# snowiow/SIFT

Measured on AMD Instinct MI355X. Metric: keypoints/sec, 1920x1080 4oct/3DoG, higher is better.
Workload: dtype f32

## Files before the change

### sift_amd/csrc/kernels_desc.hip

```cpp
#include <cstdio>

#include "common.h"
#include "hist_bins.h"

#pragma clang fp contract(off)

namespace sift_hip {

__device__ __forceinline__ int reflect_idx(int p, int n) {
    p = p < 0 ? -p : p;
    p = p >= n ? 2 * (n - 1) - p : p;
    return p < 0 ? 0 : (p >= n ? n - 1 : p);
}

__global__ __launch_bounds__(256) void w16_kernel(const float* __restrict__ level, float* __restrict__ w16,
                                                  int w, int h, const float* __restrict__ taps, int r) {
    const int img = blockIdx.x;
    const float* __restrict__ src = level + (size_t)img * (size_t)w * (size_t)h;
    const int lx = threadIdx.x & 15, ly = threadIdx.x >> 4;
    float out = 0.0f;
    if (lx < w && ly < h) {
        float sum = 0.0f;
        for (int t = 0; t <= 2 * r; ++t) {
            const int yy = reflect_idx(ly - r + t, h);
            float row = 0.0f;
            for (int s = 0; s <= 2 * r; ++s) {
                const int xx = reflect_idx(lx - r + s, w);
                row += taps[2 * r - s] * src[(size_t)yy * (size_t)w + (size_t)xx];
            }
            sum += taps[2 * r - t] * row;
        }
        out = sum;
    }
    w16[(size_t)img * 256 + (size_t)(lx + 16 * ly)] = out;
}

constexpr int kCellShift = 4;
constexpr int kW16Stride = 46;
constexpr int kW16Bias = 15 * kW16Stride + 15;
constexpr int kW16Size = 46 * kW16Stride;
struct W16Entry { float w; unsigned mask; };

typedef float f4u __attribute__((ext_vector_type(4), aligned(4)));

struct DescGridLevel {
    int w, h, dogs;
    int cw, ch, cell_base, cells_per_image;
    const float* mag;
    const float* ori;
    const float* gauss;
    const float* w16;
    int* wire_sums;
};

__device__ __forceinline__ int desc_cell_of(const DevPlan* __restrict__ plan, const FinalKp& f, int& level) {
    const int D = plan->dogs;
    level = plan->nearest_level[f.octave * D + f.index];
    const int o = level / (D + 1);
    const int w = plan->w[o], h = plan->h[o];
    const int kx = f.x, ky = f.y;
    if (kx < kRegion || kx > w - kRegion || ky < kRegion || ky > h - kRegion) return -1;
    return plan->desc_cell_base[level] + (ky >> kCellShift) * plan->desc_cw[level] + (kx >> kCellShift);
}

constexpr int kGridThreads = 1024;
constexpr int kGridLdsCells = 16384;

template <bool LDS_COUNTS>
__global__ __launch_bounds__(kGridThreads) void desc_grid_kernel(const DevPlan* __restrict__ plan, const FinalKp* __restrict__ finals,
                                                                 const int* __restrict__ final_cnt, int final_cap,
                                                                 int* __restrict__ cell_cnt, int* __restrict__ cell_off,
                                                                 FinalKp* __restrict__ pool, int pool_cap,
                                                                 long long* out_base, int compute_base,
                                                                 sift_hip_keypoint* __restrict__ kp_out, float* __restrict__ desc_out,
                                                                 long long out_cap) {
    __shared__ int s_cnt[LDS_COUNTS ? kGridLdsCells : 1];
    __shared__ int s_part[kGridThreads];
    __shared__ long long s_wsum[kGridThreads / 64];
    const int img = blockIdx.x, tid = threadIdx.x;
    const int K = final_cnt[img];
    long long my_base;
    if (compute_base) {
        long long sum = 0;
        for (int i = tid; i < img; i += kGridThreads) sum += final_cnt[i];
#pragma unroll
        for (int o = 32; o > 0; o >>= 1) sum += __shfl_down(sum, o);
        if ((tid & 63) == 0) s_wsum[tid >> 6] = sum;
        __syncthreads();
        long long t = 0;
#pragma unroll
        for (int wv = 0; wv < kGridThreads / 64; ++wv) t += s_wsum[wv];
        my_base = t;
        if (tid == 0) out_base[img] = t;
    } else {
        my_base = out_base[img];
    }
    const int cpi = plan->desc_cells_per_image;
    int* cnt = LDS_COUNTS ? s_cnt : cell_cnt + (size_t)img * (size_t)(cpi + 1);
    int* off = cell_off + (size_t)img * (size_t)(cpi + 1);
    const FinalKp* __restrict__ fin = finals + (size_t)img * (size_t)final_cap;
    for (int i = tid; i < cpi; i += kGridThreads) cnt[i] = 0;
    __syncthreads();
    for (int k = tid; k < K; k += kGridThreads) {
        const FinalKp f = fin[k];
        int level;
        const int cell = desc_cell_of(plan, f, level);
        if (cell >= 0) {
            atomicAdd(&cnt[cell], 1);
        } else {
            const long long ok = my_base + k;
            if (ok < out_cap) {
                sift_hip_keypoint r;
                r.scale = plan->dog_scale[f.octave * plan->dogs + f.index];
                r.orientation = f.orientation;
                r.x = f.x; r.y = f.y; r.octave = f.octave; r.index = f.index;
                r.filtered = 1; r.has_descriptor = 0; r.reserved = 0;
                kp_out[ok] = r;
                float4* d = reinterpret_cast<float4*>(desc_out + (size_t)ok * 128);
                for (int i = 0; i < 32; ++i) d[i] = make_float4(0.0f, 0.0f, 0.0f, 0.0f);
            }
        }
    }
    __syncthreads();
    const int chunk = (cpi + kGridThreads - 1) / kGridThreads;
    const int lo = tid * chunk, hi = min(lo + chunk, cpi);
    int sum = 0;
    for (int i = lo; i < hi; ++i) sum += cnt[i];
    s_part[tid] = sum;
    __syncthreads();
    for (int o = 1; o < kGridThreads; o <<= 1) {
        const int v = tid >= o ? s_part[tid - o] : 0;
        __syncthreads();
        s_part[tid] += v;
        __syncthreads();
    }
    int run = s_part[tid] - sum;
    for (int i = lo; i < hi; ++i) {
        const int v = cnt[i];
        off[i] = run;
        cnt[i] = run;
        run += v;
    }
    if (tid == kGridThreads - 1) off[cpi] = s_part[kGridThreads - 1];
    __syncthreads();
    FinalKp* pl = pool + (size_t)img * (size_t)pool_cap;
    for (int k = tid; k < K; k += kGridThreads) {
        FinalKp f = fin[k];
        int level;
        const int cell = desc_cell_of(plan, f, level);
        if (cell < 0) continue;
        f.cand = (uint32_t)k;
        pl[atomicAdd(&cnt[cell], 1)] = f;
    }
}

__device__ __forceinline__ int wave_min_nonneg(int v) {
    v = min(v, __builtin_amdgcn_update_dpp(0x7fffffff, v, 0xB1, 0xf, 0xf, false));
    v = min(v, __builtin_amdgcn_update_dpp(0x7fffffff, v, 0x4E, 0xf, 0xf, false));
    v = min(v, __builtin_amdgcn_update_dpp(0x7fffffff, v, 0x141, 0xf, 0xf, false));
    v = min(v, __builtin_amdgcn_update_dpp(0x7fffffff, v, 0x140, 0xf, 0xf, false));
    return min(min(__builtin_amdgcn_readlane(v, 0), __builtin_amdgcn_readlane(v, 16)),
               min(__builtin_amdgcn_readlane(v, 32), __builtin_amdgcn_readlane(v, 48)));
}

template <int Y>
__device__ __forceinline__ float quad_bcast_f(float v) {
    return __uint_as_float((unsigned)__builtin_amdgcn_mov_dpp((int)__float_as_uint(v), Y * 0x55, 0xF, 0xF, true));
}
template <int Y>
__device__ __forceinline__ unsigned quad_bcast_u(unsigned v) {
    return (unsigned)__builtin_amdgcn_mov_dpp((int)v, Y * 0x55, 0xF, 0xF, true);
}
__device__ __forceinline__ float quad_prev_f(float v) {
    return __uint_as_float((unsigned)__builtin_amdgcn_mov_dpp((int)__float_as_uint(v), 0x93 , 0xF, 0xF, true));
}

#define SIFT_HIST_SAMPLE(Y)                                                                                  \
    "v_cmp_eq_u32_sdwa vcc, %[p], %[b0] src0_sel:BYTE_" #Y " src1_sel:DWORD\n\t"                              \
    "v_add_f32_dpp %[t], %[v], %[h0] quad_perm:[" #Y "," #Y "," #Y "," #Y "] row_mask:0xf bank_mask:0xf\n\t"  \
    "v_cndmask_b32 %[h0], %[h0], %[t], vcc\n\t"                                                               \
    "v_cmp_eq_u32_sdwa vcc, %[p], %[b1] src0_sel:BYTE_" #Y " src1_sel:DWORD\n\t"                              \
    "v_add_f32_dpp %[t], %[v], %[h1] quad_perm:[" #Y "," #Y "," #Y "," #Y "] row_mask:0xf bank_mask:0xf\n\t"  \
    "v_cndmask_b32 %[h1], %[h1], %[t], vcc\n\t"
__device__ __forceinline__ void cell_histograms(const float (&val)[4], const unsigned (&bin)[4], int lane, unsigned b0, unsigned b1,
                                                float& h0, float& h1) {
    const unsigned sh = 8u * (unsigned)(lane & 3);
    unsigned pk[4];
#pragma unroll
    for (int i = 0; i < 4; ++i) pk[i] = bin[i] << sh;
    asm volatile(
        "s_nop 1\n\t"
        "v_or_b32_dpp %[p0], %[p0], %[p0] quad_perm:[1,0,3,2] row_mask:0xf bank_mask:0xf\n\t"
        "v_or_b32_dpp %[p1], %[p1], %[p1] quad_perm:[1,0,3,2] row_mask:0xf bank_mask:0xf\n\t"
        "v_or_b32_dpp %[p2], %[p2], %[p2] quad_perm:[1,0,3,2] row_mask:0xf bank_mask:0xf\n\t"
        "v_or_b32_dpp %[p3], %[p3], %[p3] quad_perm:[1,0,3,2] row_mask:0xf bank_mask:0xf\n\t"
        "v_or_b32_dpp %[p0], %[p0], %[p0] quad_perm:[2,3,0,1] row_mask:0xf bank_mask:0xf\n\t"
        "v_or_b32_dpp %[p1], %[p1], %[p1] quad_perm:[2,3,0,1] row_mask:0xf bank_mask:0xf\n\t"
        "v_or_b32_dpp %[p2], %[p2], %[p2] quad_perm:[2,3,0,1] row_mask:0xf bank_mask:0xf\n\t"
        "v_or_b32_dpp %[p3], %[p3], %[p3] quad_perm:[2,3,0,1] row_mask:0xf bank_mask:0xf\n\t"
        : [p0] "+v"(pk[0]), [p1] "+v"(pk[1]), [p2] "+v"(pk[2]), [p3] "+v"(pk[3]));
    float t;
#pragma unroll
    for (int i = 0; i < 4; ++i)
        asm volatile(
            "s_nop 1\n\t"
            SIFT_HIST_SAMPLE(0) SIFT_HIST_SAMPLE(1) SIFT_HIST_SAMPLE(2) SIFT_HIST_SAMPLE(3)
            : [h0] "+v"(h0), [h1] "+v"(h1), [t] "=&v"(t)
            : [p] "v"(pk[i]), [v] "v"(val[i]), [b0] "v"(b0), [b1] "v"(b1)
            : "vcc");
}
#undef SIFT_HIST_SAMPLE

__global__ __launch_bounds__(256, 8) void descriptor_wave_kernel(const DevPlan* __restrict__ plan, DescGridLevel lv,
                                                                 const int* __restrict__ cell_off,
                                                                 const FinalKp* __restrict__ pool, int pool_cap,
                                                                 const long long* __restrict__ out_base,
                                                                 sift_hip_keypoint* __restrict__ kp_out,
                                                                 float* __restrict__ desc_out, long long out_cap, int n_images,
                                                                 int chunks, int dbg_arg) {
    const int dbg = dbg_arg & kDiagMask;
    __shared__ __attribute__((aligned(8))) W16Entry s_w16t[kW16Size];
    __shared__ __attribute__((aligned(16))) uint2 s_list[4][64];
    __shared__ __attribute__((aligned(16))) unsigned s_keys[4][68];
    const int tid = threadIdx.x, lane = tid & 63;
    const int wave = __builtin_amdgcn_readfirstlane(tid >> 6);
    const int w = lv.w, h = lv.h, D = lv.dogs;
    const int ly = lane & 15, lx0 = (lane >> 4) * 4;
    const int tbase = kW16Bias + lx0 * kW16Stride + ly;
    const unsigned b0 = 2u * (unsigned)(lane & 3), b1 = b0 + 1u;
    for (int i = tid; i < kW16Size; i += 256) s_w16t[i] = W16Entry{0.0f, 0u};
    const int xcd = (int)blockIdx.x & 7, slot = (int)blockIdx.x >> 3, nslots = (int)gridDim.x >> 3;
    for (int unit = xcd; unit < n_images * chunks; unit += 8) {
    const int img = unit / chunks, chunk = unit - img * chunks;
    const int* __restrict__ coff = cell_off + (size_t)img * (size_t)(lv.cells_per_image + 1) + lv.cell_base;
    const int r_begin = coff[0], r_count = coff[lv.cw * lv.ch] - r_begin;
    const int e_begin = r_begin + (int)((long long)r_count * chunk / chunks), e_end = r_begin + (int)((long long)r_count * (chunk + 1) / chunks);
    if (e_begin + slot * 4 >= e_end) continue;
    __syncthreads();
    s_w16t[kW16Bias + (tid & 15) * kW16Stride + (tid >> 4)] = W16Entry{lv.w16[(size_t)img * 256 + tid], 0xffffffffu};
    __syncthreads();
    float wself[4];
#pragma unroll
    for (int i = 0; i < 4; ++i) wself[i] = s_w16t[tbase + i * kW16Stride].w;
    const size_t img_off = (size_t)img * (size_t)w * (size_t)h;
    const float* __restrict__ gm = lv.mag + img_off;
    const float* __restrict__ go = lv.ori + img_off;
    const float* __restrict__ gg = lv.gauss + img_off;
    const FinalKp* __restrict__ pl = pool + (size_t)img * (size_t)pool_cap;
    const long long obase = out_base[img];

    const int estride = nslots * 4;
    const int e0 = e_begin + slot * 4 + wave;
    struct Rec { int k; float theta; unsigned xy, oi; };
    struct Ranges { int s0, s1, s2, n0, n1, n2; };
    struct Window { f4u o, m, g; };
    auto load_rec = [&](int e) {
        const uint4 v = *reinterpret_cast<const uint4*>(&pl[min(e, e_end - 1)]);
        Rec r;
        r.k = (int)v.x; r.theta = __uint_as_float(v.y); r.xy = v.z; r.oi = v.w;
        return r;
    };
    auto load_ranges = [&](unsigned xy) {
        const int ccx = (int)(xy & 0xffffu) >> kCellShift, ccy = (int)(xy >> 16) >> kCellShift;
        const int c0 = max(ccx - 1, 0), c1 = min(ccx + 1, lv.cw - 1);
        const int y0 = max(ccy - 1, 0), y2 = min(ccy + 1, lv.ch - 1);
        const int a0 = coff[y0 * lv.cw + c0], b0_ = coff[y0 * lv.cw + c1 + 1];
        const int a1 = coff[ccy * lv.cw + c0], b1_ = coff[ccy * lv.cw + c1 + 1];
        const int a2 = coff[y2 * lv.cw + c0], b2_ = coff[y2 * lv.cw + c1 + 1];
        Ranges g;
        g.s0 = a0; g.n0 = ccy - 1 >= 0 ? b0_ - a0 : 0;
        g.s1 = a1; g.n1 = b1_ - a1;
        g.s2 = a2; g.n2 = ccy + 1 < lv.ch ? b2_ - a2 : 0;
        return g;
    };
    auto uniform_rec = [](const Rec& r) {
        Rec u;
        u.k = __builtin_amdgcn_readfirstlane(r.k);
        u.theta = __uint_as_float((unsigned)__builtin_amdgcn_readfirstlane((int)__float_as_uint(r.theta)));
        u.xy = (unsigned)__builtin_amdgcn_readfirstlane((int)r.xy);
        u.oi = (unsigned)__builtin_amdgcn_readfirstlane((int)r.oi);
        return u;
    };
    auto load_window = [&](unsigned xy) {
        size_t o = (size_t)((int)(xy >> 16) - kRegion + ly) * (size_t)w + (size_t)((int)(xy & 0xffffu) - kRegion + lx0);
        if (dbg & 8) o &= ~(size_t)3;
        if (dbg & 128) o = (size_t)ly * (size_t)w + (size_t)lx0 + (size_t)((xy >> 4) & 0xfffu) * 16u;
        Window wd;
        wd.o = (f4u)(1.0f); wd.m = (f4u)(2.0f); wd.g = (f4u)(3.0f);
        if (!(dbg & 4)) {
            wd.o = *reinterpret_cast<const f4u*>(go + o);
            wd.m = *reinterpret_cast<const f4u*>(gm + o);
            wd.g = *reinterpret_cast<const f4u*>(gg + o);
        }
        return wd;
    };
    auto entry_of = [](const Ranges& g, int i) {
        return i < g.n0 ? g.s0 + i : (i < g.n0 + g.n1 ? g.s1 + (i - g.n0) : g.s2 + (i - g.n0 - g.n1));
    };
    auto load_cand = [&](const Ranges& g) {
        const int T = g.n0 + g.n1 + g.n2;
        uint4 c = make_uint4(0u, 0u, 0u, 0u);
        if (lane < T && T <= 64) c = *reinterpret_cast<const uint4*>(&pl[entry_of(g, lane)]);
        return c;
    };
    Rec u0 = uniform_rec(load_rec(e0));
    Rec r1 = load_rec(e0 + estride);
    Ranges g0 = load_ranges(u0.xy);

    for (int e = e0; e < e_end; e += estride) {
        const uint4 c0v = load_cand(g0);
        const Window w0 = load_window(u0.xy);
        const Rec u1 = uniform_rec(r1);
        r1 = load_rec(e + 2 * estride);
        const Ranges g1 = load_ranges(u1.xy);
        const int myk = u0.k;
        const float mytheta = u0.theta;
        const unsigned myoi = u0.oi;
        const int px = (int)(u0.xy & 0xffffu), py = (int)(u0.xy >> 16);
        const int T = g0.n0 + g0.n1 + g0.n2;
        const uint4 c = c0v;
        float vo[4] = {w0.o.x, w0.o.y, w0.o.z, w0.o.w}, vm[4] = {w0.m.x, w0.m.y, w0.m.z, w0.m.w};
        const float vg[4] = {w0.g.x, w0.g.y, w0.g.z, w0.g.w};

        struct Wq { W16Entry v[4]; };
        auto weights_at = [&](int toff) {
            Wq r;
#pragma unroll
            for (int i = 0; i < 4; ++i) r.v[i] = s_w16t[tbase + toff + i * kW16Stride];
            return r;
        };
        auto apply_w = [&](unsigned qtheta_bits, const Wq& wq) {
#pragma unroll
            for (int i = 0; i < 4; ++i) {
                vo[i] = vo[i] + __uint_as_float(qtheta_bits & wq.v[i].mask);
                vm[i] = vm[i] + wq.v[i].w;
            }
        };
        auto apply = [&](unsigned qxy, float qtheta) {
            const int dx = px - (int)(qxy & 0xffffu), dy = py - (int)(qxy >> 16);
            apply_w(__float_as_uint(qtheta), weights_at(dx * kW16Stride + dy));
        };

        if (!(dbg & 1)) {
            auto precedes = [&](const uint4& c) {
                const int qx = (int)(c.z & 0xffffu), qy = (int)(c.z >> 16);
                return (int)c.x < myk && (unsigned)(qx - px + 15) < 31u && (unsigned)(qy - py + 15) < 31u;
            };
            if (T <= 64) {
                const bool pass = lane < T && precedes(c);
                const unsigned long long todo = __ballot(pass);
                const int n_prev = __popcll(todo);
                if (n_prev) {
                    unsigned* keys = s_keys[wave];
                    const int pos = (int)__builtin_amdgcn_mbcnt_hi((unsigned)(todo >> 32), __builtin_amdgcn_mbcnt_lo((unsigned)todo, 0u));
                    if (pass) keys[pos] = c.x;
                    if (lane < 4) keys[n_prev + lane] = 0xffffffffu;
                    __builtin_amdgcn_wave_barrier();
                    int rank = 0;
                    for (int ch = 0; ch < n_prev; ch += 4) {
                        const uint4 k4 = *reinterpret_cast<const uint4*>(keys + ch);
                        rank += (k4.x < c.x ? 1 : 0) + (k4.y < c.x ? 1 : 0) + (k4.z < c.x ? 1 : 0) + (k4.w < c.x ? 1 : 0);
                    }
                    uint2* list = s_list[wave];
                    if (pass) {
                        const int dx = px - (int)(c.z & 0xffffu), dy = py - (int)(c.z >> 16);
                        list[rank] = make_uint2(c.y, (unsigned)(dx * kW16Stride + dy));
                    }
                    __builtin_amdgcn_wave_barrier();
                    int r = 0;
                    for (; r + 1 < n_prev; r += 2) {
                        const uint4 q01 = *reinterpret_cast<const uint4*>(&list[r]);
                        const Wq wq0 = weights_at((int)q01.y), wq1 = weights_at((int)q01.w);
                        apply_w(q01.x, wq0);
                        apply_w(q01.z, wq1);
                    }
                    if (r < n_prev) {
                        const uint2 q0 = list[r];
                        apply_w(q0.x, weights_at((int)q0.y));
                    }
                    __builtin_amdgcn_wave_barrier();
                }
            } else {
                int last = -1;
                for (;;) {
                    int bk = 0x7fffffff;
                    unsigned bxy = 0u, bth = 0u;
                    for (int base = 0; base < T; base += 64) {
                        const int i = base + lane;
                        if (i < T) {
                            const uint4 c = *reinterpret_cast<const uint4*>(&pl[entry_of(g0, i)]);
                            if (precedes(c) && (int)c.x > last && (int)c.x < bk) { bk = (int)c.x; bxy = c.z; bth = c.y; }
                        }
                    }
                    const int m = wave_min_nonneg(bk);
                    if (m == 0x7fffffff) break;
                    const int src = (int)__builtin_ctzll(__ballot(bk == m));
                    apply((unsigned)__builtin_amdgcn_readlane((int)bxy, src), __uint_as_float((unsigned)__builtin_amdgcn_readlane((int)bth, src)));
                    last = m;
                }
            }
        }
        float val[4];
        unsigned bin[4];
#pragma unroll
        for (int i = 0; i < 4; ++i) {
            const float no = vo[i] + mytheta;
            const float nm = vm[i] + wself[i];
            val[i] = nm * vg[i];
            bin[i] = hist8_bin(no);
        }
        float h0 = 0.0f, h1 = 0.0f;
        if (!(dbg & 2)) {
            cell_histograms(val, bin, lane, b0, b1, h0, h1);
            float run = 0.0f;
            run += h0; run += h1;
            float acc = run;
#pragma unroll
            for (int step = 1; step < 4; ++step) {
                const float prev = quad_prev_f(acc);
                float t = prev;
                t += h0; t += h1;
                acc = ((lane & 3) == step) ? t : acc;
            }
            const float length = quad_bcast_f<3>(acc);
            if (!(length == 0.0f)) {
                h0 = h0 / length;
                h1 = h1 / length;
            }
        }
        const long long ok = obase + (long long)myk;
        if (ok < out_cap && !((dbg & 16) && h0 == 12345.0f)) {
            typedef float f2nt __attribute__((ext_vector_type(2)));
            __builtin_nontemporal_store((f2nt){h0, h1}, reinterpret_cast<f2nt*>(desc_out + (size_t)ok * 128 + (size_t)(2 * lane)));
            if (lv.wire_sums != nullptr) {
                const bool b0 = __float_as_uint(h0) != 0u, odd7 = (lane & 3) == 3;
                const bool b1 = !odd7 && __float_as_uint(h1) != 0u;
                const int nset = __popcll(__ballot(b0)) + __popcll(__ballot(b1));
                const unsigned long long bin7 = __ballot(odd7 && __float_as_uint(h1) != 0u);
                if (lane == 0) {
                    atomicAdd(&lv.wire_sums[1 + (ok >> 6)], nset);
                    if (bin7 != 0ull) atomicOr(&lv.wire_sums[0], 1);
                }
            }
            if (lane == 0) {
                sift_hip_keypoint r;
                r.scale = plan->dog_scale[(myoi & 0xffffu) * (unsigned)D + (myoi >> 16)];
                r.orientation = mytheta;
                r.x = (uint16_t)px; r.y = (uint16_t)py;
                r.octave = (uint16_t)(myoi & 0xffffu); r.index = (uint16_t)(myoi >> 16);
                r.filtered = 0; r.has_descriptor = 1; r.reserved = 0;
                kp_out[ok] = r;
            }
        }
        u0 = u1;
        g0 = g1;
    }
    }
}

void launch_w16(hipStream_t s, const DevPlan& plan, int level, const float* d_taps16, int radius16) {
    const int oct = level / (plan.dogs + 1);
    hipLaunchKernelGGL(w16_kernel, dim3((unsigned)plan.n_images), dim3(256), 0, s,
                       (const float*)plan.gauss[level], plan.w16[level], plan.w[oct], plan.h[oct], d_taps16,
                       radius16);
}

void launch_desc_grid(hipStream_t s, const DevPlan* d_plan, const DevPlan& plan, const FinalKp* d_final, const int* d_final_cnt,
                      int final_cap, int* d_cell_cnt, int* d_cell_off, FinalKp* d_pool, int pool_cap, long long* d_out_base,
                      bool compute_base, sift_hip_keypoint* d_kp_out, float* d_desc_out, long long out_cap) {
    if (plan.desc_cells_per_image <= kGridLdsCells)
        hipLaunchKernelGGL(desc_grid_kernel<true>, dim3((unsigned)plan.n_images), dim3(kGridThreads), 0, s, d_plan, d_final, d_final_cnt,
                           final_cap, d_cell_cnt, d_cell_off, d_pool, pool_cap, d_out_base, compute_base ? 1 : 0, d_kp_out, d_desc_out, out_cap);
    else
        hipLaunchKernelGGL(desc_grid_kernel<false>, dim3((unsigned)plan.n_images), dim3(kGridThreads), 0, s, d_plan, d_final, d_final_cnt,
                           final_cap, d_cell_cnt, d_cell_off, d_pool, pool_cap, d_out_base, compute_base ? 1 : 0, d_kp_out, d_desc_out, out_cap);
}

void launch_descriptors_wave(hipStream_t s, const DevPlan* d_plan, const DevPlan& plan, int level, const int* d_cell_off,
                             const FinalKp* d_pool, int pool_cap, const long long* d_out_base, sift_hip_keypoint* d_kp_out,
                             float* d_desc_out, long long out_cap, int dbg, int* d_wire_sums, hipEvent_t ev_start, hipEvent_t ev_stop) {
    DescGridLevel lv;
    const int oct = level / (plan.dogs + 1);
    lv.w = plan.w[oct]; lv.h = plan.h[oct]; lv.dogs = plan.dogs;
    lv.cw = plan.desc_cw[level]; lv.ch = plan.desc_ch[level]; lv.cell_base = plan.desc_cell_base[level];
    lv.cells_per_image = plan.desc_cells_per_image;
    lv.mag = plan.mag[level]; lv.ori = plan.ori[level]; lv.gauss = plan.gauss[level]; lv.w16 = plan.w16[level];
    lv.wire_sums = d_wire_sums;
    const int chunks = plan.n_images >= 8 ? 1 : 8;
    const unsigned nwg = (dbg & kDiagMask & 64) ? 512u : ((dbg & kDiagMask & 32) ? 1024u : 2048u);
    hipExtLaunchKernelGGL(descriptor_wave_kernel, dim3(nwg), dim3(256), 0, s, ev_start, ev_stop, 0, d_plan, lv, d_cell_off, d_pool, pool_cap, d_out_base,
                       d_kp_out, d_desc_out, out_cap, plan.n_images, chunks, dbg);
}

__global__ void tu_probe_desc_kernel() {}
void tu_touch_desc(hipStream_t s) { hipLaunchKernelGGL(tu_probe_desc_kernel, dim3(1), dim3(1), 0, s); }

}
```

Before: 230.4 million.

## Build per-cell orientation histograms in LDS instead of DPP compare-select chains

```diff
diff --git a/sift_amd/csrc/kernels_desc.hip b/sift_amd/csrc/kernels_desc.hip
--- a/sift_amd/csrc/kernels_desc.hip
+++ b/sift_amd/csrc/kernels_desc.hip
@@ -2,6 +2,7 @@
 
 #include "common.h"
 #include "hist_bins.h"
+#include "lds_tile.h"
 
 #pragma clang fp contract(off)
 
@@ -163,53 +164,42 @@
                min(__builtin_amdgcn_readlane(v, 32), __builtin_amdgcn_readlane(v, 48)));
 }
 
-template <int Y>
-__device__ __forceinline__ float quad_bcast_f(float v) {
-    return __uint_as_float((unsigned)__builtin_amdgcn_mov_dpp((int)__float_as_uint(v), Y * 0x55, 0xF, 0xF, true));
-}
-template <int Y>
-__device__ __forceinline__ unsigned quad_bcast_u(unsigned v) {
-    return (unsigned)__builtin_amdgcn_mov_dpp((int)v, Y * 0x55, 0xF, 0xF, true);
-}
-__device__ __forceinline__ float quad_prev_f(float v) {
-    return __uint_as_float((unsigned)__builtin_amdgcn_mov_dpp((int)__float_as_uint(v), 0x93 , 0xF, 0xF, true));
-}
-
-#define SIFT_HIST_SAMPLE(Y)                                                                                  \
-    "v_cmp_eq_u32_sdwa vcc, %[p], %[b0] src0_sel:BYTE_" #Y " src1_sel:DWORD\n\t"                              \
-    "v_add_f32_dpp %[t], %[v], %[h0] quad_perm:[" #Y "," #Y "," #Y "," #Y "] row_mask:0xf bank_mask:0xf\n\t"  \
-    "v_cndmask_b32 %[h0], %[h0], %[t], vcc\n\t"                                                               \
-    "v_cmp_eq_u32_sdwa vcc, %[p], %[b1] src0_sel:BYTE_" #Y " src1_sel:DWORD\n\t"                              \
-    "v_add_f32_dpp %[t], %[v], %[h1] quad_perm:[" #Y "," #Y "," #Y "," #Y "] row_mask:0xf bank_mask:0xf\n\t"  \
-    "v_cndmask_b32 %[h1], %[h1], %[t], vcc\n\t"
-__device__ __forceinline__ void cell_histograms(const float (&val)[4], const unsigned (&bin)[4], int lane, unsigned b0, unsigned b1,
-                                                float& h0, float& h1) {
-    const unsigned sh = 8u * (unsigned)(lane & 3);
-    unsigned pk[4];
-#pragma unroll
-    for (int i = 0; i < 4; ++i) pk[i] = bin[i] << sh;
+#define SIFT_HIST_ADD(X)                        \
+    "ds_read_b32 %[t], %[a" #X "]\n\t"          \
+    "s_waitcnt lgkmcnt(0)\n\t"                  \
+    "v_add_f32 %[t], %[v" #X "], %[t]\n\t"      \
+    "ds_write_b32 %[a" #X "], %[t]\n\t"
+#define SIFT_HIST_COLUMN(X)                                                                                \
+    SIFT_HIST_ADD(X) "s_lshl_b64 exec, exec, 1\n\t" SIFT_HIST_ADD(X) "s_lshl_b64 exec, exec, 1\n\t"        \
+    SIFT_HIST_ADD(X) "s_lshl_b64 exec, exec, 1\n\t" SIFT_HIST_ADD(X)
+typedef float f4v __attribute__((ext_vector_type(4)));
+__device__ __forceinline__ void cell_histograms(const float (&val)[4], const unsigned (&addr)[4], unsigned pair, unsigned lo, unsigned hi,
+                                                float& h0, float& h1, f4v& bins_lo, f4v& bins_hi) {
+    unsigned long long own;
+    float t;
     asm volatile(
-        "s_nop 1\n\t"
-        "v_or_b32_dpp %[p0], %[p0], %[p0] quad_perm:[1,0,3,2] row_mask:0xf bank_mask:0xf\n\t"
-        "v_or_b32_dpp %[p1], %[p1], %[p1] quad_perm:[1,0,3,2] row_mask:0xf bank_mask:0xf\n\t"
-        "v_or_b32_dpp %[p2], %[p2], %[p2] quad_perm:[1,0,3,2] row_mask:0xf bank_mask:0xf\n\t"
-        "v_or_b32_dpp %[p3], %[p3], %[p3] quad_perm:[1,0,3,2] row_mask:0xf bank_mask:0xf\n\t"
-        "v_or_b32_dpp %[p0], %[p0], %[p0] quad_perm:[2,3,0,1] row_mask:0xf bank_mask:0xf\n\t"
-        "v_or_b32_dpp %[p1], %[p1], %[p1] quad_perm:[2,3,0,1] row_mask:0xf bank_mask:0xf\n\t"
-        "v_or_b32_dpp %[p2], %[p2], %[p2] quad_perm:[2,3,0,1] row_mask:0xf bank_mask:0xf\n\t"
-        "v_or_b32_dpp %[p3], %[p3], %[p3] quad_perm:[2,3,0,1] row_mask:0xf bank_mask:0xf\n\t"
-        : [p0] "+v"(pk[0]), [p1] "+v"(pk[1]), [p2] "+v"(pk[2]), [p3] "+v"(pk[3]));
-    float t;
-#pragma unroll
-    for (int i = 0; i < 4; ++i)
-        asm volatile(
-            "s_nop 1\n\t"
-            SIFT_HIST_SAMPLE(0) SIFT_HIST_SAMPLE(1) SIFT_HIST_SAMPLE(2) SIFT_HIST_SAMPLE(3)
-            : [h0] "+v"(h0), [h1] "+v"(h1), [t] "=&v"(t)
-            : [p] "v"(pk[i]), [v] "v"(val[i]), [b0] "v"(b0), [b1] "v"(b1)
-            : "vcc");
-}
-#undef SIFT_HIST_SAMPLE
+        "v_mov_b64 %[own], 0\n\t"
+        "ds_write_b64 %[p], %[own]\n\t"
+        "s_mov_b32 exec_lo, 0x11111111\n\t"
+        "s_mov_b32 exec_hi, 0x11111111\n\t"
+        SIFT_HIST_COLUMN(0) "s_lshr_b64 exec, exec, 3\n\t"
+        SIFT_HIST_COLUMN(1) "s_lshr_b64 exec, exec, 3\n\t"
+        SIFT_HIST_COLUMN(2) "s_lshr_b64 exec, exec, 3\n\t"
+        SIFT_HIST_COLUMN(3)
+        "s_mov_b64 exec, -1\n\t"
+        "ds_read_b64 %[own], %[p]\n\t"
+        "ds_read_b128 %[blo], %[lo]\n\t"
+        "ds_read_b128 %[bhi], %[hi]\n\t"
+        "s_waitcnt lgkmcnt(0)\n\t"
+        : [own] "=&v"(own), [t] "=&v"(t), [blo] "=&v"(bins_lo), [bhi] "=&v"(bins_hi)
+        : [a0] "v"(addr[0]), [a1] "v"(addr[1]), [a2] "v"(addr[2]), [a3] "v"(addr[3]),
+          [v0] "v"(val[0]), [v1] "v"(val[1]), [v2] "v"(val[2]), [v3] "v"(val[3]), [p] "v"(pair), [lo] "v"(lo), [hi] "v"(hi)
+        : "memory", "scc");
+    h0 = __uint_as_float((unsigned)own);
+    h1 = __uint_as_float((unsigned)(own >> 32));
+}
+#undef SIFT_HIST_COLUMN
+#undef SIFT_HIST_ADD
 
 __global__ __launch_bounds__(256, 8) void descriptor_wave_kernel(const DevPlan* __restrict__ plan, DescGridLevel lv,
                                                                  const int* __restrict__ cell_off,
@@ -227,7 +217,6 @@
     const int w = lv.w, h = lv.h, D = lv.dogs;
     const int ly = lane & 15, lx0 = (lane >> 4) * 4;
     const int tbase = kW16Bias + lx0 * kW16Stride + ly;
-    const unsigned b0 = 2u * (unsigned)(lane & 3), b1 = b0 + 1u;
     for (int i = tid; i < kW16Size; i += 256) s_w16t[i] = W16Entry{0.0f, 0u};
     const int xcd = (int)blockIdx.x & 7, slot = (int)blockIdx.x >> 3, nslots = (int)gridDim.x >> 3;
     for (int unit = xcd; unit < n_images * chunks; unit += 8) {
@@ -411,18 +400,20 @@
         }
         float h0 = 0.0f, h1 = 0.0f;
         if (!(dbg & 2)) {
-            cell_histograms(val, bin, lane, b0, b1, h0, h1);
-            float run = 0.0f;
-            run += h0; run += h1;
-            float acc = run;
-#pragma unroll
-            for (int step = 1; step < 4; ++step) {
-                const float prev = quad_prev_f(acc);
-                float t = prev;
-                t += h0; t += h1;
-                acc = ((lane & 3) == step) ? t : acc;
-            }
-            const float length = quad_bcast_f<3>(acc);
+            unsigned l = (unsigned)lane;
+            asm volatile("" : "+v"(l));
+            const unsigned swz = l & 16u;
+            const unsigned hist_cell = lds_addr(s_list[wave]) + 32u * (l >> 2);
+            unsigned addr[4];
+#pragma unroll
+            for (int i = 0; i < 4; ++i) addr[i] = hist_cell + ((4u * bin[i]) ^ swz);
+            const unsigned lo = hist_cell + swz;
+            f4v b03, b47;
+            cell_histograms(val, addr, hist_cell + ((8u * (l & 3u)) ^ swz), lo, hist_cell + (swz ^ 16u), h0, h1, b03, b47);
+            __builtin_amdgcn_wave_barrier();
+            float length = 0.0f;
+            length += b03.x; length += b03.y; length += b03.z; length += b03.w;
+            length += b47.x; length += b47.y; length += b47.z; length += b47.w;
             if (!(length == 0.0f)) {
                 h0 = h0 / length;
                 h1 = h1 / length;
```

Result: no change. 230.8 million (median of 4 runs) (+0.2%).
